# rvp-group/srrg2_slam_interfaces

Measured on AMD Instinct MI355X. Metric: icp_iterations_per_sec, higher is better.
Workload: dtype f32; 1 GPU; C2: SE(3) point-to-plane AlignerSlice, 100000-pt synthetic cloud pair per GPU, 10 ICP iterations per compute(), gated NN 0.25 m + normal gate, Cauchy 0.05; points=100000, alignments_total=1, all_success=True, last_status=0, last_num_inliers=99432, parallelism=single GPU

## Files before the change

### srrg2_slam_interfaces_amd/csrc/aligner_host.hip

```cpp
#include <algorithm>
#include <cmath>
#include <cstdio>
#include <cstdlib>
#include <chrono>
#include <cstring>
#include <string>
#include <vector>

#include "det_math.h"
#include "kernels.h"

#include "host_util.h"

namespace srrg2amd {
thread_local std::string g_err;
int fail(int code, const std::string& msg) {
  g_err = msg;
  return code;
}
}

namespace {

using srrg2amd::DevBuf;
// ... 57 lines not shown
  DevBuf<unsigned long long> zbuf;
  DevBuf<int> queue;
  DevBuf<int> qcount;
  float prior_Z[12]{};
  bool has_prior = false;
  void release() {
    if (qprobe_host) (void) hipHostFree(qprobe_host);
    qprobe_host = nullptr;
    qprobe_cap  = 0;
    if (bbox_host) (void) hipHostFree(bbox_host);
    bbox_host     = nullptr;
    bbox_host_cap = 0;
    if (ms_probs_host) (void) hipHostFree(ms_probs_host);
    ms_probs_host     = nullptr;
    ms_probs_host_cap = 0;
    fixed_raw.release(); fixed_nrm_raw.release(); fixed_sorted.release(); fixed_nrm_sorted.release();
    cell_start.release(); cursor.release(); scan_sums.release(); scalars.release(); pos_of.release();
    list_start.release(); list_sums.release(); list_ent.release(); list_box.release(); list_offs.release(); list_hdr.release();
    moving.release(); moving_nrm.release(); pinf.release();
    moving_raw.release(); moving_nrm_raw.release(); ms_counts.release(); ms_cursor.release(); ms_sums.release();
    ms_bb.release(); ms_probs.release();
    corr_fixed.release(); gcorr.release(); gcorr_off.release(); gcorr_stat.release(); prev_n.release(); prev_pos.release(); prev_f.release(); prev_m.release(); corr_resp.release(); corr_stat.release(); partials.release(); zbuf.release(); queue.release(); qcount.release(); bbox_rows.release();
  }
};

}

struct srrg2_aligner_s {
  int kind = 0, dim = 3, dof = 6, tsize = 12, device = 0;
  hipStream_t stream = nullptr;
  static constexpr int MAX_PARTS = 8;
  hipStream_t pstream[MAX_PARTS]{};
  int cu_count          = 256;
  int fused_grid_max    = 130000;
  hipEvent_t ev_staged  = nullptr;
  hipEvent_t ev_records = nullptr;
  bool records_unsynced = false;
  int parts_dirty       = 0;
  int batch_parts       = 0;
  int part_begin[MAX_PARTS + 1]{};
  srrg2_aligner_params params{10, 10, 0, 0};
  srrg2_reduce_fn reduce_fn = nullptr;
  void* reduce_user         = nullptr;
  long long shard_total     = 0;
  bool has_term = false;
  srrg2_termination_params term{5, 20, 20, 20, 0.2f};
  std::vector<Slice*> slices;
  float X[12]{};
  int status = SRRG2_FAIL;
  int K = 1;
  DevBuf<ProblemDev> probs;
  DevBuf<ProblemState> states;
  DevBuf<ProblemOut> outs;
  DevBuf<srrg2_iteration_stats> stats;
  DevBuf<float> guesses;
  DevBuf<unsigned long long> pub;
  DevBuf<unsigned> pub_epoch;
  DevBuf<CtlParams> ctl_dev;
  DevBuf<char> staging;
  DevBuf<float4> pair_raw, pair_nrm_raw, pair_sorted, pair_nrm_sorted;
  DevBuf<int> pair_cell_start, pair_cursor, pair_scan_sums, pair_pos_of;
  DevBuf<unsigned> pair_rows;
  DevBuf<ProblemDev> pair_fprobs;
  DevBuf<GridDev> pair_grids;
  DevBuf<char> pair_staging;
  unsigned* pair_rows_host = nullptr; size_t pair_rows_host_cap = 0;
// ... 662 lines not shown
  const srrg2_aligner_tuning& tn = a->tuning;
  C.probe_it      = tn.queue_probe_iteration;
  if (a->params.max_iterations <= C.probe_it + 3 || K > 4) C.probe_it = -1;
  bool small = false;
  {
    int ncue = 0, fc = -1;
    for (int si = 0; si < nslices; ++si)
      if (a->slices[si]->cfg.kind != SRRG2_SLICE_PRIOR) {
        if (fc < 0) fc = si;
        ++ncue;
      }
    const int small_max = tn.small_max_points;
    small = ncue == 1 && a->slices[fc]->cfg.finder == SRRG2_FINDER_NN_GATED && max_nm <= small_max &&
            a->timeline_path.empty() && !a->reduce_fn;
    const bool priors_launch = nslices > ncue && (tn.fused_control == 2 || nslices - ncue > 2);
    if (small && !pairs && (priors_launch || tn.fused_control == 0 || a->params.max_iterations < 2)) small = max_nm <= 640;
    if (small && !pairs && !(priors_launch || tn.fused_control == 0 || a->params.max_iterations < 2)) {
      const Slice* sfc = a->slices[fc];
      const int sl     = tn.search_lists;
      const bool lists = sl >= 2 || (sl == 1 && K > 4) || (sl < 0 && (K > 4 || sfc->grid_computes >= 1 || sfc->lists_tried));
      small            = !lists && max_nm <= 384;
    }
  }
  const int fast_from = tn.fast_from_iteration;
  bool fuse = false;
  auto fast_ppt_of = [&](int k_launch) {
    return tn.fast_points_per_thread > 0 ? tn.fast_points_per_thread : (k_launch >= (fuse ? 16 : 64) ? 2 : 1);
  };
  const int fast_min = tn.fast_min_points;
  const bool fast_gather = tn.fast_gather >= 0 ? tn.fast_gather != 0 : K > 4;
  const bool fast_batch_queue = tn.fast_batch_queue != 0;
  const int lds_tile = pairs ? 0 : (tn.lds_tile >= 0 ? tn.lds_tile : (K > 4 ? 1 : 0));
  const int search_lists = tn.search_lists;
  const int search_team_knob = tn.search_team;
  std::vector<char> cnl((size_t) std::max(nslices, 1), 0);
  std::vector<SliceDev> sdev((size_t) nslices);
  int first_cue = -1;
  for (int si = 0; si < nslices; ++si) {
    Slice* s     = a->slices[si];
    SliceCtl& sc = C.slices[si];
    sc.kind                     = s->cfg.kind;
    sc.min_num_correspondences  = s->cfg.min_num_correspondences;
    sc.robust_kind              = s->cfg.robustifier;
    sc.robust_thr               = s->cfg.robustifier_chi_threshold;
    sc.gate                     = s->cfg.finder_max_distance;
    sc.has_prior                = s->has_prior ? 1 : 0;
    sc.prior_sets_initial_guess = s->cfg.prior_sets_initial_guess;
    std::memcpy(sc.prior_Z, s->prior_Z, sizeof(sc.prior_Z));
    std::memcpy(sc.prior_info, s->cfg.prior_information_diag, sizeof(sc.prior_info));
    sc.partials  = nullptr;
    sc.finder    = s->cfg.finder;
    sc.K0        = s->cfg.camera_matrix[0];
    sc.K4        = s->cfg.camera_matrix[4];
    sc.umax      = proj_extent(s->cfg.image_cols, s->cfg.camera_matrix[2]);
    sc.vmax      = proj_extent(s->cfg.image_rows, s->cfg.camera_matrix[5]);
    sc.depth_min = s->cfg.depth_min;
    sc.pinf_bits = nullptr;
    sc.ninf_bits = nullptr;
    if (s->cfg.kind == SRRG2_SLICE_PRIOR) continue;
    if (first_cue < 0) first_cue = si;
    int nm_max_s = 0;
    for (int k = 0; k < K; ++k) nm_max_s = std::max(nm_max_s, all[(size_t) si * K + k].nm);
    const int queue_min = tn.queue_min_points;
    const bool want_lists = search_lists >= 2 || (search_lists == 1 && K > 4) ||
                            (search_lists < 0 && (K > 4 || s->grid_computes >= 1 || s->lists_tried));
    if (!pairs) s->grid_computes++;
    if (s->cfg.finder == SRRG2_FINDER_NN_GATED && !small && want_lists && !pairs) {
// ... 450 lines not shown
                                     a->states.p, K, nm_max, a->stream);
          sdev[si].zbuf_parity ^= 1;
        } else {
          SliceDev sd = sdev[si];
          const bool fast = (slot0 > 0 || (it >= fast_from && it >= 1)) && nm_max >= fast_min;
          if (!queue_on[si] || (s->fast_queue_only && !fast)) {
            sd.queue  = nullptr;
            sd.qcount = nullptr;
          }
          for (int h = 0; h < nhalves; ++h) {
            sd.prob0 = h0[h];
            if (fuse) {
              if (!fused_pass(slot0, it)) sd.fc.pub = nullptr;
              sd.fc.ctl   = a->ctl_dev.p + h;
              sd.fc.epoch = epoch;
              sd.partials = slot_buffer(s, pround);
              sd.fc.prev_partials = slot_buffer(s, pround + 2);
              sd.fc.zero_partials = slot_buffer(s, pround + 1);
              sd.fc.prior         = (slot0 > 0 || it > 0) ? 1 : 0;
              if (it == 0) sd.fc.prior_mask = 0;
            }
            const ProblemDev* pt = a->probs.p + (size_t) si * K;
            hipStream_t hs = hstream[h];
            const int Kh   = hn[h];
            const bool first_pass_init = fold_init && slot0 == 0 && it == 0 && si == first_cue;
            if (pairs && fast)
              srrg2amd::launch_icp_step_fast_pairs(a->dim, plane, sd, pair_grids, pt, a->states.p, Kh, nm_max, fast_ppt_of(Kh),
                                                   fast_gather, hs);
            else if (pairs)
              srrg2amd::launch_icp_step_pairs(a->dim, plane, sd, pair_grids, pt, a->states.p, Kh, nm_max, hs);
            else if (fast)
              srrg2amd::launch_icp_step_fast(a->dim, plane, sd, pt, a->states.p, Kh, nm_max, fast_ppt_of(Kh), fast_gather, hs);
            else if (cnl[(size_t) si] && !sd.queue)
              srrg2amd::launch_icp_step_cnl(a->dim, plane, sd, s->lists_host, pt, a->states.p, Kh, nm_max,
                                            search_team_knob > 0 ? search_team_knob : ((K <= 4 && slot0 == 0 && it == 0) ? 4 : 1), hs,
                                            first_pass_init ? &Ch[h] : nullptr, first_pass_init ? &fold_inl : nullptr,
                                            first_pass_init && !fold_bat.empty() ? &fold_bat[(size_t) h] : nullptr);
            else if (!sd.queue && lds_tile > 0 && !small)
              srrg2amd::launch_icp_step_tile(a->dim, plane, sd, pt, a->states.p, Kh, nm_max, lds_tile == 2 ? 504 : 416, hs);
            else
              srrg2amd::launch_icp_step(a->dim, plane, sd, pt, a->states.p, Kh, nm_max, hs, first_pass_init ? &Ch[h] : nullptr,
                                        first_pass_init ? &fold_inl : nullptr);
            if (split) control(it, last_phase, h);
          }
        }
        if (a->profile) HIP_TRY(hipEventRecord(e1, a->stream));
      }
      if (!split) control(it, last_phase, 0);
      ++epoch;
      ++pround;
    }
    return 0;
  };
  if (small) {
    final_launched = true;
  } else {
    if ((rc = run_phase(0, !a->params.enable_inlier_only_runs))) return rc;
    if (a->params.enable_inlier_only_runs) {
      for (int h = 0; h < nhalves; ++h) {
        Ch[h].epoch = epoch + 1;
        srrg2amd::launch_icp_post(Ch[h], a->states.p, a->stats.p, hstream[h]);
      }
      ++epoch;
      if ((rc = run_phase(a->params.max_iterations, true))) return rc;
    }
  }
  if (!final_launched)
    for (int h = 0; h < nhalves; ++h)
      srrg2amd::launch_icp_finalize(Ch[h], a->states.p, a->stats.p, a->outs_host, a->stats_host,
                                    !a->params.enable_inlier_only_runs , hstream[h]);
// ... 256 lines not shown
  c->finder_normal_cos = -2.f;
  c->finder_cell_size = 0.f;
  identity(variable_kind, c->sensor_in_robot);
  for (int i = 0; i < 6; ++i) c->prior_information_diag[i] = variable_kind == SRRG2_SE2_RIGHT ? 100.f : 1.f;
  c->prior_sets_initial_guess = 1;
}

int srrg2_aligner_create(int variable_kind, int device, srrg2_aligner_h* out) {
  if (!out || variable_kind < 0 || variable_kind > 2) return fail(SRRG2_E_INVALID, "create: bad arguments");
  int n = 0;
  hipError_t e = hipGetDeviceCount(&n);
  if (e != hipSuccess || n <= 0)
    return fail(SRRG2_E_NO_DEVICE, "create: no HIP device visible (this library has no CPU fallback)");
  if (device < 0 || device >= n) return fail(SRRG2_E_INVALID, "create: bad device ordinal");
  srrg2_aligner* a = new srrg2_aligner();
  a->kind   = variable_kind;
  a->dim    = variable_kind == SRRG2_SE2_RIGHT ? 2 : 3;
  a->dof    = variable_kind == SRRG2_SE2_RIGHT ? 3 : 6;
  a->tsize  = variable_kind == SRRG2_SE2_RIGHT ? 9 : 12;
  a->device = device;
  identity(variable_kind, a->X);
  tuning_from_environment(&a->tuning);
  if (const char* tl = std::getenv("SRRG2_AMD_TIMELINE")) a->timeline_path = tl;
  a->hosttime = std::getenv("SRRG2_AMD_HOSTTIME") != nullptr;
  if (const char* fg = std::getenv("SRRG2_AMD_FUSED_GRID_MAX")) a->fused_grid_max = std::atoi(fg);
  bool ok = hipSetDevice(device) == hipSuccess && hipStreamCreateWithFlags(&a->stream, hipStreamNonBlocking) == hipSuccess;
  a->pstream[0] = a->stream;
  ok = ok && hipEventCreateWithFlags(&a->ev_staged, hipEventDisableTiming) == hipSuccess;
  ok = ok && hipEventCreateWithFlags(&a->ev_records, hipEventDisableTiming) == hipSuccess;
  if (ok && (hipDeviceGetAttribute(&a->cu_count, hipDeviceAttributeMultiprocessorCount, device) != hipSuccess || a->cu_count <= 0)) {
    (void) hipGetLastError();
    a->cu_count = 256;
  }
  if (!ok) {
    for (int p = 0; p < srrg2_aligner::MAX_PARTS; ++p)
      if (a->pstream[p]) (void) hipStreamDestroy(a->pstream[p]);
    delete a;
    return fail(SRRG2_E_HIP, "create: cannot create stream");
  }
  *out = a;
  return 0;
}

int srrg2_aligner_destroy(srrg2_aligner_h a) {
  if (!a) return 0;
  (void) hipSetDevice(a->device);
  for (int p = 0; p < srrg2_aligner::MAX_PARTS; ++p)
    if (a->pstream[p]) (void) hipStreamSynchronize(a->pstream[p]);
  for (Slice* s : a->slices) {
    s->release();
    delete s;
  }
  a->probs.release(); a->states.release(); a->outs.release(); a->stats.release(); a->guesses.release();
  a->pub.release(); a->pub_epoch.release(); a->ctl_dev.release();
  a->staging.release();
  a->pair_raw.release(); a->pair_nrm_raw.release(); a->pair_sorted.release(); a->pair_nrm_sorted.release();
  a->pair_cell_start.release(); a->pair_cursor.release(); a->pair_scan_sums.release(); a->pair_pos_of.release();
  a->pair_rows.release(); a->pair_fprobs.release(); a->pair_grids.release(); a->pair_staging.release();
  if (a->pair_rows_host) (void) hipHostFree(a->pair_rows_host);
  if (a->pair_fprobs_host) (void) hipHostFree(a->pair_fprobs_host);
  if (a->pair_grids_host) (void) hipHostFree(a->pair_grids_host);
  if (a->outs_host) (void) hipHostFree(a->outs_host);
  if (a->stats_host) (void) hipHostFree(a->stats_host);
  if (a->guesses_host) (void) hipHostFree(a->guesses_host);
  if (a->probs_host) (void) hipHostFree(a->probs_host);
  for (auto& ev : a->prof_events) {
// ... 818 lines not shown
```

### srrg2_slam_interfaces_amd/csrc/kernels.h

```cpp
#pragma once
#include "device_types.h"

namespace srrg2amd {

void launch_ingest(const float* src, int stride_floats, int n, int dim, float4* dst, unsigned* maxabs_bits,
                   int finite_per_point, hipStream_t s);
void launch_ingest_batch(const float* src, int stride_floats, const ProblemDev* probs, int K, int max_nm, int dim,
                         float4* dst, unsigned* maxabs_bits, int finite_per_point, hipStream_t s);
void launch_bbox(const float4* pts, int n, unsigned* mn, unsigned* mx, int* nvalid, hipStream_t s);
void launch_ingest_bbox(const float* src, int stride_floats, int n, int dim, float4* dst, unsigned* maxabs_bits, unsigned* mn,
                        unsigned* mx, int* nvalid, hipStream_t s, unsigned* ticket, unsigned* host_out, unsigned seq,
                        unsigned* block_out , unsigned* clear_after);
#define INGEST_BBOX_MAX_BLOCKS 512
void launch_grid_count(const GridDev& g, const float4* pts, int n, int* counts, hipStream_t s);
void launch_count_nonzero(const int* counts, int n, int* out, hipStream_t s);
int scan_num_blocks(int n);
void launch_exclusive_scan(int* data, int n, int* block_sums, int* grand_total, hipStream_t s, int* copy = nullptr);
void launch_grid_scatter(const GridDev& g, const float4* pts, const float4* nrm, int n, int* cursor, float4* out_pts,
                         float4* out_nrm, int* pos_of, hipStream_t s);
void launch_cnl_build(const GridDev& g, const GridLists& L, const int4* offs, int noffs, int* list_start, uint2* box_at,
                      uint4* ent, hipStream_t s);
void launch_icp_step_cnl(int dim, bool plane, const SliceDev& S, const GridLists& GL, const ProblemDev* probs,
                         ProblemState* states, int K, int max_nm, int team, hipStream_t s, const CtlParams* init_C = nullptr,
                         const InitInline* init_inl = nullptr, const InitBatch* init_bat = nullptr);
bool launch_msort_local(const float* src, int sf, const float* nsrc, int nsf, const ProblemDev* probs, int K, int dim, int kbits,
                        int aniso, int segments, int max_nm, float4* out_pts, float4* out_nrm, unsigned* maxabs_bits,
                        hipStream_t s);
void launch_msort(const float4* pts, const float4* nrm, const ProblemDev* probs, int K, int max_nm, int kbits, int aniso,
                  unsigned* bb, int* counts, int* cursor, int* scan_sums, int* scan_total, float4* out_pts,
                  float4* out_nrm, hipStream_t s);
void launch_icp_step(int dim, bool plane, const SliceDev& S, const ProblemDev* probs, ProblemState* states, int K,
                     int max_nm, hipStream_t s, const CtlParams* init_C = nullptr, const InitInline* init_inl = nullptr);
void launch_icp_step_tile(int dim, bool plane, const SliceDev& S, const ProblemDev* probs, ProblemState* states, int K,
                          int max_nm, int cap, hipStream_t s);
void launch_icp_step_fast(int dim, bool plane, const SliceDev& S, const ProblemDev* probs, ProblemState* states, int K,
                          int max_nm, int ppt, bool gather, hipStream_t s);
void launch_icp_outputs(int dim, bool plane, const SliceDev& S, const ProblemDev* probs, const ProblemState* states, int K,
                        int max_nm, hipStream_t s);
int icp_step_blocks(int max_nm);
int icp_queue_blocks(int max_nm, int K);
void launch_proj_step_pack(const SliceDev* slices, const ProblemDev* const* probs, int nslices, ProblemState* states, int K,
                           int max_nm, hipStream_t s);
void launch_proj_records(const SliceDev& S0, const SliceDev& S, const ProblemDev* probs0, const ProblemDev* probs,
                         ProblemState* states, int K, int max_nm, bool rebuild, hipStream_t s);
void launch_proj_step_fused(const SliceDev* slices, const ProblemDev* const* probs, int nslices, ProblemState* states, int K,
                            int max_nm, hipStream_t s,
                            const CtlParams* init_C = nullptr, const InitInline* init_inl = nullptr, ProblemDev* probs_base = nullptr);
void launch_corr_step(int dim, bool plane, const SliceDev& S, const ProblemDev* probs, ProblemState* states, int K,
                      int max_ncorr, hipStream_t s);
void launch_proj_step(bool repro, const SliceDev& S, const ProblemDev* probs, ProblemState* states, int K, int max_nm,
                      hipStream_t s);
void launch_icp_init(const CtlParams& C, const ProblemDev* probs_host, ProblemDev* probs, ProblemState* states,
                     const float* guesses_host, int tsize, hipStream_t s, bool pairs = false);
bool make_init_inline(const CtlParams& C, const ProblemDev* probs_host, const float* guesses_host, int tsize, InitInline* inl);
void launch_icp_control(const CtlParams& C, ProblemState* states, srrg2_iteration_stats* stats, hipStream_t s);
void launch_icp_final_wave_pack(const SliceDev* slices, const ProblemDev* const* probs, int nslices, ProblemState* states,
                                srrg2_iteration_stats* stats, ProblemOut* outs_host, srrg2_iteration_stats* stats_host,
// ... 25 lines not shown
```

### srrg2_slam_interfaces_amd/csrc/kernels.hip

```cpp
#include <cstdlib>
#include <algorithm>

#include "kernels.h"

#include <type_traits>

#include "det_math.h"

#include "device_util.h"

namespace {

#define FX_MAGIC 6755399441055744.0
#define FX_MAGIC_BITS 0x4338000000000000ll
__device__ __forceinline__ long long fx_bits(double biased) { return __double_as_longlong(biased) - FX_MAGIC_BITS; }

__device__ __forceinline__ unsigned long long key_min(unsigned long long a, unsigned long long b) {
  double r;
  asm("v_min_f64 %0, %1, %2" : "=v"(r) : "v"(__longlong_as_double((long long) a)), "v"(__longlong_as_double((long long) b)));
  return (unsigned long long) __double_as_longlong(r);
}

template <int DIM>
__device__ __forceinline__ float cand_d2(const float4 f, float qx, float qy, float qz) {
  const float dx = f.x - qx, dy = f.y - qy;
  float d2       = dx * dx + dy * dy;
  if (DIM == 3) {
    const float dz = f.z - qz;
    d2             = d2 + dz * dz;
  }
  return d2;
}

template <int DIM>
__device__ __forceinline__ void test_candidate(const float4 f, float qx, float qy, float qz, bool valid,
                                               unsigned long long& bkey) {
// ... 1705 lines not shown
    }
    const int team = lane >> 4;
    const int mine = team == 0 ? src[0] : (team == 1 ? src[1] : (team == 2 ? src[2] : src[3]));
    const int from = mine >= 0 ? mine : lane;
    float wbest, wexcl2;
    int widx, wpos;
    const int sr_from = __shfl(r2, from);
    coop_scan<DIM, 16>(g, lane, wlds[wid].coop, __shfl(qx, from), __shfl(qy, from), __shfl(qz, from), __shfl(cx, from),
                       __shfl(cy, from), __shfl(cz, from), mine >= 0 ? sr_from : -1, __shfl(ball2, from), wbest, widx, wpos,
                       wexcl2);
#pragma unroll
    for (int t = 0; t < 4; ++t) {
      const float rb = __shfl(wbest, 16 * t), re = __shfl(wexcl2, 16 * t);
      const int ri = __shfl(widx, 16 * t);
      if (lane == src[t]) {
        excl_wide = sqrtf(re) * 0.99999f;
        if (rb < best || (rb == best && ri < bidx)) {
          best = rb;
          bidx = ri;
        }
      }
    }
  }
  if (excl_wide != 0.f || r2 != 0) excl = excl_wide;
  long long acc[ACC_N];
#pragma unroll
  for (int a = 0; a < ACC_N; ++a) acc[a] = 0;
  finish_point<DIM, PLANE>(S, T, rk, thr, kk, scale, inrange, active, gi, oi, p, qx, qy, qz, best, bidx, bpos, excl, skipped,
                           pf, pn, pnm, use_prior && S.use_normal_gate, acc);
  block_reduce_store<NW>(acc, S.partials, prob, tile, nullptr);
}

#ifdef SRRG2_PASS_TIMELINE
__device__ unsigned long long g_pass_ts[16 * 512 * 8];
#define PASS_TS_ANY(epoch, k)                       \
  do {                                                                                                 \
    if ((threadIdx.x & 63) == 0 && (epoch) >= 0 && (epoch) < 16 && blockIdx.y < 512 && blockIdx.x == 0) \
      g_pass_ts[(((epoch) * 512) + blockIdx.y) * 8 + (k)] = wall_clock64();                            \
  } while (0)
#define PASS_TS_W(epoch, k, dep)              \
  do {                                                                                                 \
    if (threadIdx.x == 0 && (epoch) >= 0 && (epoch) < 16 && blockIdx.x == 0) {                         \
      unsigned long long t_ = wall_clock64();                                                          \
      if ((dep) != (dep)) t_ = 0;         \
      g_pass_ts[(((epoch) * 512) + 0) * 8 + (k)] = t_;                                                  \
    }                                                                                                  \
  } while (0)
#define PASS_TS(epoch, k)                                                                              \
  do {                                                                                                 \
    if (threadIdx.x == 0 && (epoch) >= 0 && (epoch) < 16 && blockIdx.y < 512 && blockIdx.x == 0)       \
      g_pass_ts[(((epoch) * 512) + blockIdx.y) * 8 + (k)] = wall_clock64();                            \
  } while (0)
#else
#define PASS_TS(epoch, k) do { } while (0)
#define PASS_TS_ANY(epoch, k) do { } while (0)
#define PASS_TS_W(epoch, k, dep) do { } while (0)
#endif
namespace {

__device__ float robust_weight(int kind, float thr, float chi, bool& kernelized);
template <bool PAIRS = false>
__device__ __forceinline__ int slice_exponent(const CtlParams& C, const SliceCtl& s, int prob, int nm, const float* X);
template <bool ONLY_INLINE, bool PAIRS = false>
__device__ __forceinline__ void init_problem_thread0(const CtlParams& C, int prob, const ProblemDev* probs_host, ProblemDev* probs,
                                                     ProblemState* states, const float* guesses_host, int tsize,
                                                     const InitInline& inl, unsigned (*init_gran)[PUB_SLICE_GRANULES]);

__device__ __forceinline__ double rl_d(double v, int k) {
  const int lo = __builtin_amdgcn_readlane(__double2loint(v), k);
  const int hi = __builtin_amdgcn_readlane(__double2hiint(v), k);
  return __hiloint2double(hi, lo);
}
__device__ __forceinline__ long long rl_ll(long long v, int k) {
  const int lo = __builtin_amdgcn_readlane((int) (unsigned) v, k);
  const int hi = __builtin_amdgcn_readlane((int) (unsigned) ((unsigned long long) v >> 32), k);
  return (long long) (((unsigned long long) (unsigned) hi << 32) | (unsigned) lo);
}
__device__ __forceinline__ float rl_f(float v, int k) { return __int_as_float(__builtin_amdgcn_readlane(__float_as_int(v), k)); }
__device__ __forceinline__ double wave_max_d(double v) {
#pragma unroll
  for (int off = 32; off >= 1; off >>= 1) {
    const double o = __shfl_xor(v, off);
    v              = o > v ? o : v;
  }
// ... 1227 lines not shown
        }
      }
    }
  };
  constexpr bool defer = PPT == 1 && FUSED;
  float d_qx = 0.f, d_qy = 0.f, d_qz = 0.f, d_best = INFINITY;
  bool d_valid = false;
#pragma unroll
  for (int k = 0; k < PPT; ++k) {
    const bool active = inr[k] && finite3(p[k].x, p[k].y, p[k].z);
    float qx, qy, qz, px, py, pz;
    transform_point<DIM>(T, p[k], qx, qy, qz);
    transform_point<DIM>(Tprev, p[k], px, py, pz);
    const float ex = qx - px, ey = qy - py, ez = qz - pz;
    const float dl   = __builtin_amdgcn_sqrtf((ex * ex + ey * ey) + ez * ez);
    const bool hasp  = __float_as_int(pf[k].w) != NO_MATCH;
    unsigned long long k1 = NO_KEY;
    test_candidate<DIM>(pf[k], qx, qy, qz, true, k1);
    const float best = key_best(k1);
    const float d1   = __builtin_amdgcn_sqrtf(best);
    const float rhs  = pm[k] * 0.99999f;
    const bool ca   = hasp && (d1 * 1.00001f + dl * 1.00001f < rhs);
    const bool cc   = !hasp && pm[k] > 0.f && (gate_r * 1.00001f + dl * 1.00001f < rhs);
    const bool have = active && (ca || cc);
    const float excl = pm[k] * 0.9999999f - dl * 1.00001f;
    const float pad  = fminf(2.f * dl, PAD_CAP * g.h) + PAD_MIN * g.h;
    const float rr   = (d1 + pad) * 1.00001f;
    const float r2box = hasp ? fminf(rr * rr, gfar) : gfar;
    open_ball2[k]     = (active && !have) ? r2box : -1.f;
    any_open |= active && !have;
#ifdef SRRG2_PASS_TIMELINE
    if constexpr (FUSED) {
      if (active && !have && S.fc.epoch >= 0 && S.fc.epoch < 16 && blockIdx.x == 0) {
        unsigned long long* c = &g_pass_ts[((size_t) S.fc.epoch * 512 + 500) * 8];
        const float gap = (pm[k] - d1) / g.h;
        atomicAdd(&c[0], 1ull);
        if (!hasp) atomicAdd(&c[1], 1ull);
        else if (gap < 1e-4f) atomicAdd(&c[2], 1ull);
        else if (gap < 0.0202f) atomicAdd(&c[3], 1ull);
        else atomicAdd(&c[4], 1ull);
        if (dl > 1e-3f * g.h) atomicAdd(&c[5], 1ull);
        if (pm[k] <= 0.f) atomicAdd(&c[6], 1ull);
      }
    }
#endif
    if constexpr (defer) {
      d_qx = qx; d_qy = qy; d_qz = qz; d_best = best; d_valid = have && ca;
    } else if (k == 0) {
      linearize(std::true_type{}, acc, have && ca, p[k], pf[k], pn[k], pnm[k], qx, qy, qz, best);
    } else {
      linearize(std::false_type{}, acc, have && ca, p[k], pf[k], pn[k], pnm[k], qx, qy, qz, best);
    }
    if (have) S.prev_m[gi_[k]] = excl;
  }
  if constexpr (defer) {
    {
      if (__any(any_open)) {
        float sbest[PPT], sexcl[PPT];
        int sidx[PPT], spos[PPT];
        search_open(sbest, sidx, sexcl, spos);
        const bool open = open_ball2[0] >= 0.f;
        const bool same = open && sidx[0] != NO_MATCH && sidx[0] == __float_as_int(pf[0].w);
        if (open && !same) {
          pf[0] = make_float4(0.f, 0.f, 0.f, __int_as_float(NO_MATCH));
          pn[0] = make_float4(0.f, 0.f, 0.f, 0.f);
          if (sidx[0] != NO_MATCH) {
            spos[0] = g.pos_of[sidx[0]];
// ... 78 lines not shown
    transform_point<DIM>(T, p[k], qx, qy, qz);
    if (k == 0)
      linearize(std::true_type{}, acc2, open, p[k], fk, nk, pnm[k], qx, qy, qz, sbest[k]);
    else
      linearize(std::false_type{}, acc2, open, p[k], fk, nk, pnm[k], qx, qy, qz, sbest[k]);
    if (open) {
      S.prev_m[gi_[k]] = sexcl[k];
      if (!same) {
        S.prev_pos[gi_[k]] = sidx[k] != NO_MATCH ? spos[k] : -1;
        if (!GATHER) {
          S.prev_f[gi_[k]] = fk;
          if (PLANE || ngate) S.prev_n[gi_[k]] = nk;
        }
      }
    }
  }
  block_reduce_store_biased<1>(acc2, S.partials, prob, tile, PPT);
  if constexpr (FUSED) PASS_TS_ANY(S.fc.epoch, 4);
  block_reduce_store_biased<4, 2>(acc, S.partials, prob, tile, PPT);
  if constexpr (FUSED) PASS_TS(S.fc.epoch, 3);
}

template <int DIM, bool PLANE, int PPT, bool GATHER, int FUSED>
__global__ __launch_bounds__(256) void k_icp_step_fast(SliceDev S, const ProblemDev* __restrict__ probs,
                                                       ProblemState* __restrict__ states) {
  icp_step_fast_body<DIM, PLANE, PPT, GATHER, FUSED>(S, probs, states);
}
template <int DIM, bool PLANE, int PPT, bool GATHER>
__global__ __launch_bounds__(256) void k_icp_step_fast_pairs(SliceDev S, const GridDev* __restrict__ grids,
                                                             const ProblemDev* __restrict__ probs, ProblemState* __restrict__ states) {
  S.grid = grids[blockIdx.y + S.prob0];
  icp_step_fast_body<DIM, PLANE, PPT, GATHER, 0>(S, probs, states);
}
template <int DIM, bool PLANE, int TEAM, int FUSED>
__device__ __forceinline__ void cnl_pass_body(const SliceDev& S, const GridLists& GL, const ProblemDev* __restrict__ probs,
                                              ProblemState* __restrict__ states, const CtlParams* Ci = nullptr,
                                              const InitInline* inl = nullptr, const InitBatch* bat = nullptr) {
  constexpr int NW  = 4;
  constexpr int PPB = NW * 64 / TEAM;
  const int prob    = (FUSED ? blockIdx.x : blockIdx.y) + S.prob0;
  PassView pv;
  if constexpr (!FUSED) {
    pass_view_legacy(S, &states[prob], pv);
    if (pv.stop) return;
  } else if constexpr (FUSED != 3) {
    PASS_TS(S.fc.epoch, 0);
    fused_control_if_due<DIM, FUSED == 2>(S, states, prob);
  }
  ProblemDev pd;
  if constexpr (FUSED == 3) {
    if (bat)
      pd = bat->pd[prob - Ci->prob0];
    else
      pd = inl->pd[S.slice_idx];
  } else {
    pd = probs[prob];
  }
  const int tile      = FUSED ? blockIdx.y : blockIdx.x;
  const bool tail_wg = FUSED == 3 && tile == (int) gridDim.y - 1;
  if (tile * PPB >= pd.nm && (!FUSED || (FUSED == 3 ? !tail_wg : tile != 0))) return;
  float T[12], Tprev[12];
  double scale;
  int rk;
  bool use_prior;
  if constexpr (!FUSED) {
    load_T(pv.T, T);
    load_T(pv.Tprev, Tprev);
    scale     = dm::pow2(pv.kexp);
    rk        = (pv.phase1 && S.robust_kind != SRRG2_ROBUST_NONE) ? (int) SRRG2_ROBUST_CLAMP : S.robust_kind;
    use_prior = pv.prior;
  } else {
    use_prior = S.fc.prior != 0;
  }
  const float thr    = S.robust_thr;
  const float kk     = S.variable_kind == SRRG2_SE3_QUAT_RIGHT ? 2.f : 1.f;
  const GridDev& g   = S.grid;
  const float gfar = use_prior ? g.gate2_ext : g.gate2;

  __shared__ CnlWave wlds[NW];

  const int i        = tile * PPB + (int) threadIdx.x / TEAM;
  const int lane     = threadIdx.x & 63;
  const int wid      = threadIdx.x >> 6;
  const bool leader  = (threadIdx.x & (TEAM - 1)) == 0;
  const bool inrange = i < pd.nm;
  const int gi       = pd.moff + (inrange ? i : 0);
  float4 p           = make_float4(0.f, 0.f, 0.f, 0.f);
  float4 pf          = make_float4(0.f, 0.f, 0.f, __int_as_float(NO_MATCH));
  float4 pn          = make_float4(0.f, 0.f, 0.f, 0.f);
  float4 pnm         = make_float4(0.f, 0.f, 0.f, 0.f);
  float pm           = 0.f;
  if (inrange) {
    p = S.mpts[gi];
    if (use_prior) {
      pm = S.prev_m[gi];
      if (S.use_normal_gate) pnm = S.mnrm[gi];
      if (S.gather_prev) {
        const int ppos = S.prev_pos[gi];
        if (ppos >= 0 && ppos < S.grid.n) {
          pf = S.grid.pts[ppos];
          if (PLANE || S.use_normal_gate) pn = S.grid.nrm[ppos];
        }
      } else {
        pf = S.prev_f[gi];
        if (PLANE || S.use_normal_gate) pn = S.prev_n[gi];
      }
    }
  }
  if constexpr (FUSED) {
    if constexpr (FUSED == 3) {
      pass_view_init<DIM>(S, *Ci, *inl, prob, pd.nm, pv, bat);
      if (tail_wg && threadIdx.x < 64)
        fused_init_tail(*Ci, *inl, prob, const_cast<ProblemDev*>(probs) - (size_t) S.slice_idx * Ci->K, states, bat, pv, S.slice_idx);
    } else {
      pass_view_fused<DIM, FUSED == 2>(S, states, prob, pv);
    }
    if (pv.stop || tile * PPB >= pd.nm) return;
    load_T(pv.T, T);
    load_T(pv.Tprev, Tprev);
    scale = dm::pow2(pv.kexp);
    rk    = (pv.phase1 && S.robust_kind != SRRG2_ROBUST_NONE) ? (int) SRRG2_ROBUST_CLAMP : S.robust_kind;
  }
  const bool has_prev = __float_as_int(pf.w) != NO_MATCH;
  const bool active   = inrange && finite3(p.x, p.y, p.z);
  float qx = 0.f, qy = 0.f, qz = 0.f;
  float best = INFINITY;
  int bidx = NO_MATCH;
  float excl = 0.f, r2box = INFINITY;
  bool skipped = false;
  if (active) {
    transform_point<DIM>(T, p, qx, qy, qz);
    if (use_prior && has_prev) {
      unsigned long long k1 = NO_KEY;
      test_candidate<DIM>(pf, qx, qy, qz, true, k1);
      float px, py, pz;
      transform_point<DIM>(Tprev, p, px, py, pz);
      const float ex = qx - px, ey = qy - py, ez = qz - pz;
      const float dl = sqrtf((ex * ex + ey * ey) + ez * ez);
      const float d1 = sqrtf(key_best(k1));
      if (d1 * 1.00001f + dl * 1.00001f < pm * 0.99999f) {
        skipped = true;
        best    = key_best(k1);
        bidx    = key_idx(k1);
        excl    = pm * 0.9999999f - dl * 1.00001f;
      } else {
        const float pad = fminf(2.f * dl, PAD_CAP * g.h) + PAD_MIN * g.h;
        const float rr  = (d1 + pad) * 1.00001f;
        r2box           = fminf(rr * rr, gfar);
      }
    } else if (use_prior && !has_prev && pm > 0.f) {
// ... 98 lines not shown
    if (!use_prior && found) nmk = S.mnrm[gi];
    float dot;
    if constexpr (DIM == 3) {
      const float rx = (T[0] * nmk.x + T[1] * nmk.y) + T[2] * nmk.z;
      const float ry = (T[4] * nmk.x + T[5] * nmk.y) + T[6] * nmk.z;
      const float rz = (T[8] * nmk.x + T[9] * nmk.y) + T[10] * nmk.z;
      dot            = (nf.x * rx + nf.y * ry) + nf.z * rz;
    } else {
      const float rx = T[0] * nmk.x + T[1] * nmk.y;
      const float ry = T[4] * nmk.x + T[5] * nmk.y;
      dot            = nf.x * rx + nf.y * ry;
    }
    found = found && dot > S.normal_cos;
  }
  long long acc[ACC_N];
  {
    float J[ROWS][D], er[ROWS];
    point_rows<DIM, PLANE>(T, kk, p, qx, qy, qz, fm, nf, J, er);
    (void) factor_accumulate_flat<D, ROWS, true>(J, er, found, rk, thr, scale, acc);
  }
  if (inrange && leader) {
    if (!skipped) {
      S.prev_pos[gi] = has ? bpos : -1;
      if (!S.gather_prev) {
        S.prev_f[gi] = fm;
        if (PLANE || ngate) S.prev_n[gi] = nf;
      }
    }
    S.prev_m[gi] = excl;
  }
  block_reduce_store_biased<NW>(acc, S.partials, prob, tile, 1);
  if constexpr (FUSED) PASS_TS(S.fc.epoch, 3);
}
template <int DIM, bool PLANE, int TEAM, int FUSED>
__global__ __launch_bounds__(256) void k_icp_step_cnl(SliceDev S, GridLists GL, const ProblemDev* __restrict__ probs,
                                                      ProblemState* __restrict__ states) {
  cnl_pass_body<DIM, PLANE, TEAM, FUSED>(S, GL, probs, states);
}
template <int DIM, bool PLANE, int TEAM>
__global__ __launch_bounds__(256) void k_icp_step_cnl_init(SliceDev S, GridLists GL, CtlParams C, InitInline inl,
                                                           ProblemDev* __restrict__ probs, ProblemState* __restrict__ states) {
  cnl_pass_body<DIM, PLANE, TEAM, 3>(S, GL, probs, states, &C, &inl);
}
template <int DIM, bool PLANE, int TEAM>
__global__ __launch_bounds__(256) void k_icp_step_cnl_init_batch(SliceDev S, GridLists GL, CtlParams C, InitBatch B,
                                                                 ProblemDev* __restrict__ probs, ProblemState* __restrict__ states) {
  const InitInline none{};
  cnl_pass_body<DIM, PLANE, TEAM, 3>(S, GL, probs, states, &C, &none, &B);
}

template <int DIM, bool PLANE>
__global__ __launch_bounds__(256) void k_icp_outputs(SliceDev S, const ProblemDev* __restrict__ probs,
                                                     const ProblemState* __restrict__ states) {
  constexpr int D    = DIM == 3 ? 6 : 3;
  constexpr int ROWS = PLANE ? 1 : DIM;
  const int prob     = blockIdx.y + S.prob0;
  const ProblemState* st = &states[prob];
  const ProblemDev pd    = probs[prob];
  const int i            = blockIdx.x * blockDim.x + threadIdx.x;
  if (i >= pd.nm) return;
  const int gi  = pd.moff + i;
  int match     = -1;
  float resp    = 0.f;
  uint8_t fstat = SRRG2_FACTOR_SUPPRESSED;
  const float4 p = S.mpts[gi];
  if (st->npasses > 0 && finite3(p.x, p.y, p.z)) {
    float4 f = make_float4(0.f, 0.f, 0.f, __int_as_float(NO_MATCH));
    int fpos = -1;
    if (S.gather_prev) {
      fpos = S.prev_pos[gi];
      if (fpos >= 0 && fpos < S.grid.n) f = S.grid.pts[fpos];
    } else {
      f = S.prev_f[gi];
    }
    if (__float_as_int(f.w) != NO_MATCH) {
      float T[12];
      load_T(st->Tlast[S.slice_idx], T);
      float qx, qy, qz;
      transform_point<DIM>(T, p, qx, qy, qz);
      unsigned long long k1 = NO_KEY;
      test_candidate<DIM>(f, qx, qy, qz, true, k1);
// ... 1523 lines not shown
    static unsigned long long zero[N];
    if (hipMemcpyToSymbol(HIP_SYMBOL(counters), zero, sizeof(zero)) != hipSuccess) return -1;
  }
  return 0;
}
#endif
#ifdef SRRG2_PASS_TIMELINE
extern "C" int srrg2_amd_debug_pass_timeline(unsigned long long* out, int reset) {
  return debug_counters(g_pass_ts, out, reset);
}
#endif
#ifdef SRRG2_CNL_STATS
extern "C" int srrg2_amd_debug_cnl_stats(unsigned long long* out, int reset) {
  return debug_counters(g_cnl_stats, out, reset);
}
#endif
#ifdef SRRG2_TILE_STATS
extern "C" int srrg2_amd_debug_tile_stats(unsigned long long* out, int reset) {
  return debug_counters(g_tile_stats, out, reset);
}
#endif

void launch_icp_step_tile(int dim, bool plane, const SliceDev& S, const ProblemDev* probs, ProblemState* states, int K,
                          int max_nm, int cap, hipStream_t s) {
  if (K <= 0 || max_nm <= 0) return;
  const dim3 grid(icp_step_blocks(max_nm), K);
  with_dim_plane(dim, plane, [&](auto D, auto P) {
    with_value<504, 416>(cap > 450, [&](auto CAP) {
      hipLaunchKernelGGL((k_icp_step_tile<D(), P(), CAP()>), grid, dim3(256), 0, s, S, probs, states);
    });
  });
}

void launch_icp_step_cnl(int dim, bool plane, const SliceDev& S, const GridLists& GL, const ProblemDev* probs,
                         ProblemState* states, int K, int max_nm, int team, hipStream_t s, const CtlParams* init_C,
                         const InitInline* init_inl, const InitBatch* init_bat) {
  if (K <= 0) return;
  ProblemDev* pw = const_cast<ProblemDev*>(probs);
  auto tiles_of = [&](auto TEAM) { return (max_nm * TEAM() + 255) / 256; };
  if (S.fc.pub && init_C && init_bat) {
    with_value<4, 1>(team >= 4, [&](auto TEAM) {
      const dim3 grid(K, tiles_of(TEAM) + 1);
      with_dim_plane(dim, plane, [&](auto D, auto P) {
        hipLaunchKernelGGL((k_icp_step_cnl_init_batch<D(), P(), TEAM()>), grid, dim3(256), 0, s, S, GL, *init_C, *init_bat, pw,
                           states);
      });
    });
    return;
  }
  if (S.fc.pub && init_C) {
    with_value<4, 1>(team >= 4, [&](auto TEAM) {
      const dim3 grid(K, tiles_of(TEAM) + 1);
      with_dim_plane(dim, plane, [&](auto D, auto P) {
        hipLaunchKernelGGL((k_icp_step_cnl_init<D(), P(), TEAM()>), grid, dim3(256), 0, s, S, GL, *init_C, *init_inl, pw,
                           states);
      });
    });
    return;
  }
  if (max_nm <= 0) return;
  auto pass = [&](auto FUSED) __attribute__((always_inline)) {
    with_value<4, 1>(team >= 4, [&](auto TEAM) {
      const dim3 grid = FUSED() ? dim3(K, tiles_of(TEAM)) : dim3(tiles_of(TEAM), K);
      with_dim_plane(dim, plane, [&](auto D, auto P) {
        hipLaunchKernelGGL((k_icp_step_cnl<D(), P(), TEAM(), FUSED()>), grid, dim3(256), 0, s, S, GL, probs, states);
      });
    });
  };
  if (S.fc.pub && S.fc.prior_mask)
    pass(int_c<2>{});
  else if (S.fc.pub)
    pass(int_c<1>{});
  else
    pass(int_c<0>{});
}

void launch_icp_step_fast(int dim, bool plane, const SliceDev& S, const ProblemDev* probs, ProblemState* states, int K,
                          int max_nm, int ppt, bool gather, hipStream_t s) {
  if (K <= 0 || max_nm <= 0) return;
  auto pass = [&](auto PPT, auto GATHER, auto FUSED) __attribute__((always_inline)) {
    const int tiles = (max_nm + 256 * PPT() - 1) / (256 * PPT());
    const dim3 grid = FUSED() ? dim3(K, tiles) : dim3(tiles, K);
    with_dim_plane(dim, plane, [&](auto D, auto P) {
      hipLaunchKernelGGL((k_icp_step_fast<D(), P(), PPT(), GATHER(), FUSED()>), grid, dim3(256), 0, s, S, probs, states);
    });
  };
  if (S.fc.pub && S.fc.prior_mask) {
    with_value<true, false>(gather, [&](auto G) { pass(int_c<1>{}, G, int_c<2>{}); });
    return;
  }
  if (S.fc.pub) {
    with_value<true, false>(gather, [&](auto G) {
      with_value<2, 1>(ppt >= 2, [&](auto PPT) { pass(PPT, G, int_c<1>{}); });
    });
    return;
  }
  with_value<true, false>(gather, [&](auto G) {
    if (ppt >= 4)
      pass(int_c<4>{}, G, int_c<0>{});
    else
      with_value<2, 1>(ppt >= 2, [&](auto PPT) { pass(PPT, G, int_c<0>{}); });
  });
  if (S.queue) launch_icp_queue(dim, plane, S, probs, states, K, max_nm, s);
}

void launch_icp_outputs(int dim, bool plane, const SliceDev& S, const ProblemDev* probs, const ProblemState* states, int K,
                        int max_nm, hipStream_t s) {
// ... 162 lines not shown
```

Before: 59320 iterations/s.

## Plan mixed-team search tiles to fill resident GPU capacity per ICP iteration

Adds a tile planner that splits the correspondence-search grid into tiles with 4, 2, or 1 lanes per point. It sizes the split against the number of resident workgroups, taken from an occupancy query, so the whole pass fits in one wave of blocks. The automatic lane choice now uses 2-lane teams for early iterations beyond the first, where it previously used 1-lane teams. The aim is better GPU utilisation for single-problem 100k-point searches, at the cost of extra template instantiations, more branching, and an occupancy query at setup.

```diff
diff --git a/srrg2_slam_interfaces_amd/csrc/aligner_host.hip b/srrg2_slam_interfaces_amd/csrc/aligner_host.hip
--- a/srrg2_slam_interfaces_amd/csrc/aligner_host.hip
+++ b/srrg2_slam_interfaces_amd/csrc/aligner_host.hip
@@ -113,6 +113,7 @@
   static constexpr int MAX_PARTS = 8;
   hipStream_t pstream[MAX_PARTS]{};
   int cu_count          = 256;
+  srrg2amd::SearchCapacity search_capacity;
   int fused_grid_max    = 130000;
   hipEvent_t ev_staged  = nullptr;
   hipEvent_t ev_records = nullptr;
@@ -841,7 +842,13 @@
   const bool fast_batch_queue = tn.fast_batch_queue != 0;
   const int lds_tile = pairs ? 0 : (tn.lds_tile >= 0 ? tn.lds_tile : (K > 4 ? 1 : 0));
   const int search_lists = tn.search_lists;
-  const int search_team_knob = tn.search_team;
+  const int search_lanes_knob          = tn.search_team & 0xff;
+  const long long search_capacity_knob = tn.search_team >> 8;
+  int first_pass_lanes = 0;
+  auto search_lanes_auto = [&](int run, int it) {
+    if (K > 4 || run != 0) return 1;
+    return it == 0 ? 4 : (it == 1 || (it == 2 && first_pass_lanes == 2)) ? 2 : 1;
+  };
   std::vector<char> cnl((size_t) std::max(nslices, 1), 0);
   std::vector<SliceDev> sdev((size_t) nslices);
   int first_cue = -1;
@@ -1358,10 +1365,16 @@
             else if (fast)
               srrg2amd::launch_icp_step_fast(a->dim, plane, sd, pt, a->states.p, Kh, nm_max, fast_ppt_of(Kh), fast_gather, hs);
             else if (cnl[(size_t) si] && !sd.queue)
-              srrg2amd::launch_icp_step_cnl(a->dim, plane, sd, s->lists_host, pt, a->states.p, Kh, nm_max,
-                                            search_team_knob > 0 ? search_team_knob : ((K <= 4 && slot0 == 0 && it == 0) ? 4 : 1), hs,
-                                            first_pass_init ? &Ch[h] : nullptr, first_pass_init ? &fold_inl : nullptr,
-                                            first_pass_init && !fold_bat.empty() ? &fold_bat[(size_t) h] : nullptr);
+            {
+              const int lanes = search_lanes_knob > 0 ? search_lanes_knob : search_lanes_auto(slot0, it);
+              const int plan_lanes = (K <= 4 && lanes > 1) ? (lanes >= 4 ? 4 : 2) : 0;
+              const int used = srrg2amd::launch_icp_step_cnl(
+                a->dim, plane, sd, s->lists_host, pt, a->states.p, Kh, nm_max, lanes >= 4 ? 4 : 1, hs,
+                first_pass_init ? &Ch[h] : nullptr, first_pass_init ? &fold_inl : nullptr,
+                first_pass_init && !fold_bat.empty() ? &fold_bat[(size_t) h] : nullptr, plan_lanes, search_lanes_knob == 0,
+                search_capacity_knob, &a->search_capacity);
+              if (slot0 == 0 && it == 0) first_pass_lanes = used;
+            }
             else if (!sd.queue && lds_tile > 0 && !small)
               srrg2amd::launch_icp_step_tile(a->dim, plane, sd, pt, a->states.p, Kh, nm_max, lds_tile == 2 ? 504 : 416, hs);
             else
@@ -1684,6 +1697,7 @@
     (void) hipGetLastError();
     a->cu_count = 256;
   }
+  a->search_capacity.cu_count = a->cu_count;
   if (!ok) {
     for (int p = 0; p < srrg2_aligner::MAX_PARTS; ++p)
       if (a->pstream[p]) (void) hipStreamDestroy(a->pstream[p]);
diff --git a/srrg2_slam_interfaces_amd/csrc/kernels.h b/srrg2_slam_interfaces_amd/csrc/kernels.h
--- a/srrg2_slam_interfaces_amd/csrc/kernels.h
+++ b/srrg2_slam_interfaces_amd/csrc/kernels.h
@@ -20,9 +20,14 @@
                          float4* out_nrm, int* pos_of, hipStream_t s);
 void launch_cnl_build(const GridDev& g, const GridLists& L, const int4* offs, int noffs, int* list_start, uint2* box_at,
                       uint4* ent, hipStream_t s);
-void launch_icp_step_cnl(int dim, bool plane, const SliceDev& S, const GridLists& GL, const ProblemDev* probs,
-                         ProblemState* states, int K, int max_nm, int team, hipStream_t s, const CtlParams* init_C = nullptr,
-                         const InitInline* init_inl = nullptr, const InitBatch* init_bat = nullptr);
+struct SearchCapacity {
+  int cu_count = 256;
+  int blocks_per_cu[2][4] = {{-1, -1, -1, -1}, {-1, -1, -1, -1}};
+};
+int launch_icp_step_cnl(int dim, bool plane, const SliceDev& S, const GridLists& GL, const ProblemDev* probs,
+                        ProblemState* states, int K, int max_nm, int team, hipStream_t s, const CtlParams* init_C = nullptr,
+                        const InitInline* init_inl = nullptr, const InitBatch* init_bat = nullptr, int plan_lanes = 0,
+                        bool plan_whole = false, long long plan_capacity = 0, SearchCapacity* cap = nullptr);
 bool launch_msort_local(const float* src, int sf, const float* nsrc, int nsf, const ProblemDev* probs, int K, int dim, int kbits,
                         int aniso, int segments, int max_nm, float4* out_pts, float4* out_nrm, unsigned* maxabs_bits,
                         hipStream_t s);
diff --git a/srrg2_slam_interfaces_amd/csrc/kernels.hip b/srrg2_slam_interfaces_amd/csrc/kernels.hip
--- a/srrg2_slam_interfaces_amd/csrc/kernels.hip
+++ b/srrg2_slam_interfaces_amd/csrc/kernels.hip
@@ -1,7 +1,9 @@
+#include <climits>
 #include <cstdlib>
 #include <algorithm>
 
 #include "kernels.h"
+#include "search_plan.h"
 
 #include <type_traits>
 
@@ -1773,24 +1775,25 @@
 }
 
 #ifdef SRRG2_PASS_TIMELINE
-__device__ unsigned long long g_pass_ts[16 * 512 * 8];
+#define PASS_TS_WGS 2048
+__device__ unsigned long long g_pass_ts[16 * PASS_TS_WGS * 8];
 #define PASS_TS_ANY(epoch, k)                       \
   do {                                                                                                 \
-    if ((threadIdx.x & 63) == 0 && (epoch) >= 0 && (epoch) < 16 && blockIdx.y < 512 && blockIdx.x == 0) \
-      g_pass_ts[(((epoch) * 512) + blockIdx.y) * 8 + (k)] = wall_clock64();                            \
+    if ((threadIdx.x & 63) == 0 && (epoch) >= 0 && (epoch) < 16 && blockIdx.y < PASS_TS_WGS - 1 && blockIdx.x == 0) \
+      g_pass_ts[(((epoch) * PASS_TS_WGS) + blockIdx.y) * 8 + (k)] = wall_clock64();                            \
   } while (0)
 #define PASS_TS_W(epoch, k, dep)              \
   do {                                                                                                 \
     if (threadIdx.x == 0 && (epoch) >= 0 && (epoch) < 16 && blockIdx.x == 0) {                         \
       unsigned long long t_ = wall_clock64();                                                          \
       if ((dep) != (dep)) t_ = 0;         \
-      g_pass_ts[(((epoch) * 512) + 0) * 8 + (k)] = t_;                                                  \
+      g_pass_ts[(((epoch) * PASS_TS_WGS) + 0) * 8 + (k)] = t_;                                                  \
     }                                                                                                  \
   } while (0)
 #define PASS_TS(epoch, k)                                                                              \
   do {                                                                                                 \
-    if (threadIdx.x == 0 && (epoch) >= 0 && (epoch) < 16 && blockIdx.y < 512 && blockIdx.x == 0)       \
-      g_pass_ts[(((epoch) * 512) + blockIdx.y) * 8 + (k)] = wall_clock64();                            \
+    if (threadIdx.x == 0 && (epoch) >= 0 && (epoch) < 16 && blockIdx.y < PASS_TS_WGS - 1 && blockIdx.x == 0)       \
+      g_pass_ts[(((epoch) * PASS_TS_WGS) + blockIdx.y) * 8 + (k)] = wall_clock64();                            \
   } while (0)
 #else
 #define PASS_TS(epoch, k) do { } while (0)
@@ -3084,7 +3087,7 @@
 #ifdef SRRG2_PASS_TIMELINE
     if constexpr (FUSED) {
       if (active && !have && S.fc.epoch >= 0 && S.fc.epoch < 16 && blockIdx.x == 0) {
-        unsigned long long* c = &g_pass_ts[((size_t) S.fc.epoch * 512 + 500) * 8];
+        unsigned long long* c = &g_pass_ts[((size_t) S.fc.epoch * PASS_TS_WGS + PASS_TS_WGS - 1) * 8];
         const float gap = (pm[k] - d1) / g.h;
         atomicAdd(&c[0], 1ull);
         if (!hasp) atomicAdd(&c[1], 1ull);
@@ -3229,10 +3232,11 @@
   S.grid = grids[blockIdx.y + S.prob0];
   icp_step_fast_body<DIM, PLANE, PPT, GATHER, 0>(S, probs, states);
 }
-template <int DIM, bool PLANE, int TEAM, int FUSED>
+template <int DIM, bool PLANE, int TEAM, int FUSED, bool PLANNED = false>
 __device__ __forceinline__ void cnl_pass_body(const SliceDev& S, const GridLists& GL, const ProblemDev* __restrict__ probs,
                                               ProblemState* __restrict__ states, const CtlParams* Ci = nullptr,
-                                              const InitInline* inl = nullptr, const InitBatch* bat = nullptr) {
+                                              const InitInline* inl = nullptr, const InitBatch* bat = nullptr,
+                                              CnlWave* plan_wlds = nullptr, const int plan_tile = 0, const int plan_first = 0) {
   constexpr int NW  = 4;
   constexpr int PPB = NW * 64 / TEAM;
   const int prob    = (FUSED ? blockIdx.x : blockIdx.y) + S.prob0;
@@ -3243,6 +3247,8 @@
   } else if constexpr (FUSED != 3) {
     PASS_TS(S.fc.epoch, 0);
     fused_control_if_due<DIM, FUSED == 2>(S, states, prob);
+  } else {
+    PASS_TS(S.fc.epoch, 0);
   }
   ProblemDev pd;
   if constexpr (FUSED == 3) {
@@ -3253,9 +3259,10 @@
   } else {
     pd = probs[prob];
   }
-  const int tile      = FUSED ? blockIdx.y : blockIdx.x;
+  const int tile      = PLANNED ? plan_tile : (int) (FUSED ? blockIdx.y : blockIdx.x);
+  const auto first_of = [&]() { return PLANNED ? plan_first : tile * PPB; };
   const bool tail_wg = FUSED == 3 && tile == (int) gridDim.y - 1;
-  if (tile * PPB >= pd.nm && (!FUSED || (FUSED == 3 ? !tail_wg : tile != 0))) return;
+  if (first_of() >= pd.nm &&(!FUSED || (FUSED == 3 ? !tail_wg : tile != 0))) return;
   float T[12], Tprev[12];
   double scale;
   int rk;
@@ -3274,9 +3281,15 @@
   const GridDev& g   = S.grid;
   const float gfar = use_prior ? g.gate2_ext : g.gate2;
 
-  __shared__ CnlWave wlds[NW];
-
-  const int i        = tile * PPB + (int) threadIdx.x / TEAM;
+  CnlWave* wlds;
+  if constexpr (PLANNED) {
+    wlds = plan_wlds;
+  } else {
+    __shared__ CnlWave own_wlds[NW];
+    wlds = own_wlds;
+  }
+
+  const int i        = first_of() + (int) threadIdx.x / TEAM;
   const int lane     = threadIdx.x & 63;
   const int wid      = threadIdx.x >> 6;
   const bool leader  = (threadIdx.x & (TEAM - 1)) == 0;
@@ -3312,7 +3325,7 @@
     } else {
       pass_view_fused<DIM, FUSED == 2>(S, states, prob, pv);
     }
-    if (pv.stop || tile * PPB >= pd.nm) return;
+    if (pv.stop || first_of() >= pd.nm) return;
     load_T(pv.T, T);
     load_T(pv.Tprev, Tprev);
     scale = dm::pow2(pv.kexp);
@@ -3477,6 +3490,23 @@
   block_reduce_store_biased<NW>(acc, S.partials, prob, tile, 1);
   if constexpr (FUSED) PASS_TS(S.fc.epoch, 3);
 }
+struct TilePlan {
+  int t4, t2;
+};
+template <int DIM, bool PLANE, int FUSED>
+__device__ __forceinline__ void cnl_pass_tiles(const SliceDev& S, const GridLists& GL, const ProblemDev* __restrict__ probs,
+                                               ProblemState* __restrict__ states, const TilePlan& plan, const CtlParams* Ci = nullptr,
+                                               const InitInline* inl = nullptr, const InitBatch* bat = nullptr) {
+  __shared__ CnlWave wlds[4];
+  const int tile = FUSED ? blockIdx.y : blockIdx.x;
+  const int t4 = plan.t4, t2 = plan.t2;
+  if (tile < t4)
+    cnl_pass_body<DIM, PLANE, 4, FUSED, true>(S, GL, probs, states, Ci, inl, bat, wlds, tile, tile * 64);
+  else if (tile < t4 + t2)
+    cnl_pass_body<DIM, PLANE, 2, FUSED, true>(S, GL, probs, states, Ci, inl, bat, wlds, tile, t4 * 64 + (tile - t4) * 128);
+  else
+    cnl_pass_body<DIM, PLANE, 1, FUSED, true>(S, GL, probs, states, Ci, inl, bat, wlds, tile, t4 * 64 + t2 * 128 + (tile - t4 - t2) * 256);
+}
 template <int DIM, bool PLANE, int TEAM, int FUSED>
 __global__ __launch_bounds__(256) void k_icp_step_cnl(SliceDev S, GridLists GL, const ProblemDev* __restrict__ probs,
                                                       ProblemState* __restrict__ states) {
@@ -3492,6 +3522,17 @@
                                                                  ProblemDev* __restrict__ probs, ProblemState* __restrict__ states) {
   const InitInline none{};
   cnl_pass_body<DIM, PLANE, TEAM, 3>(S, GL, probs, states, &C, &none, &B);
+}
+template <int DIM, bool PLANE, int FUSED>
+__global__ __launch_bounds__(256) void k_icp_step_cnl_plan(SliceDev S, GridLists GL, const ProblemDev* __restrict__ probs,
+                                                           ProblemState* __restrict__ states, TilePlan plan) {
+  cnl_pass_tiles<DIM, PLANE, FUSED>(S, GL, probs, states, plan);
+}
+template <int DIM, bool PLANE>
+__global__ __launch_bounds__(256) void k_icp_step_cnl_init_plan(SliceDev S, GridLists GL, CtlParams C, InitInline inl,
+                                                                ProblemDev* __restrict__ probs, ProblemState* __restrict__ states,
+                                                                TilePlan plan) {
+  cnl_pass_tiles<DIM, PLANE, 3>(S, GL, probs, states, plan, &C, &inl);
 }
 
 template <int DIM, bool PLANE>
@@ -5081,13 +5122,70 @@
   });
 }
 
-void launch_icp_step_cnl(int dim, bool plane, const SliceDev& S, const GridLists& GL, const ProblemDev* probs,
-                         ProblemState* states, int K, int max_nm, int team, hipStream_t s, const CtlParams* init_C,
-                         const InitInline* init_inl, const InitBatch* init_bat) {
-  if (K <= 0) return;
+static long long cnl_plan_capacity(int dim, bool plane, int kind, SearchCapacity& cap) {
+  int& per_cu = cap.blocks_per_cu[plane ? 1 : 0][kind];
+  if (per_cu < 0) {
+    int n = 0;
+    hipError_t e = hipErrorUnknown;
+    with_dim_plane(dim, plane, [&](auto D, auto P) {
+      if (kind == 3)
+        e = hipOccupancyMaxActiveBlocksPerMultiprocessor(&n, k_icp_step_cnl_init_plan<D(), P()>, 256, 0);
+      else if (kind == 2)
+        e = hipOccupancyMaxActiveBlocksPerMultiprocessor(&n, k_icp_step_cnl_plan<D(), P(), 2>, 256, 0);
+      else if (kind == 1)
+        e = hipOccupancyMaxActiveBlocksPerMultiprocessor(&n, k_icp_step_cnl_plan<D(), P(), 1>, 256, 0);
+      else
+        e = hipOccupancyMaxActiveBlocksPerMultiprocessor(&n, k_icp_step_cnl_plan<D(), P(), 0>, 256, 0);
+    });
+    if (e != hipSuccess) {
+      (void) hipGetLastError();
+      n = 0;
+    }
+    per_cu = n > 6 ? n - 1 : n;
+  }
+  return (long long) per_cu * cap.cu_count;
+}
+
+int launch_icp_step_cnl(int dim, bool plane, const SliceDev& S, const GridLists& GL, const ProblemDev* probs,
+                        ProblemState* states, int K, int max_nm, int team, hipStream_t s, const CtlParams* init_C,
+                        const InitInline* init_inl, const InitBatch* init_bat, int plan_lanes, bool plan_whole,
+                        long long plan_capacity, SearchCapacity* cap) {
+  if (K <= 0) return 0;
   ProblemDev* pw = const_cast<ProblemDev*>(probs);
   auto tiles_of = [&](auto TEAM) { return (max_nm * TEAM() + 255) / 256; };
-  if (S.fc.pub && init_C && init_bat) {
+  const bool init_b = S.fc.pub && init_C && init_bat, init_1 = S.fc.pub && init_C && !init_bat;
+  if (plan_lanes > 1 && cap && !init_b && (init_1 || max_nm > 0)) {
+    const int kind = init_1 ? 3 : (S.fc.pub && S.fc.prior_mask) ? 2 : S.fc.pub ? 1 : 0;
+    const long long resident = plan_capacity > 0 ? plan_capacity : cnl_plan_capacity(dim, plane, kind, *cap);
+    const long long room = std::min(resident - (kind == 3 ? K : 0), 65534ll * K);
+    SearchTiles t{0, 0, 0};
+    bool planned = true;
+    if (plan_whole) {
+      planned = false;
+      for (int l = plan_lanes >= 4 ? 4 : 2; l > 1 && !planned; l >>= 1) {
+        t       = plan_search_tiles(max_nm, K, room, l);
+        planned = (l == 4 ? t.t2 + t.t1 : t.t4 + t.t1) == 0;
+      }
+    } else {
+      t = plan_search_tiles(max_nm, K, room, plan_lanes);
+    }
+    const TilePlan tp{t.t4, t.t2};
+    SliceDev Sp = S;
+    if (resident > 0 && resident < (long long) INT_MAX) Sp.fc.first_round = (int) resident;
+    if (planned) with_dim_plane(dim, plane, [&](auto D, auto P) {
+      if (kind == 3)
+        hipLaunchKernelGGL((k_icp_step_cnl_init_plan<D(), P()>), dim3(K, t.tiles() + 1), dim3(256), 0, s, Sp, GL, *init_C,
+                           *init_inl, pw, states, tp);
+      else if (kind == 2)
+        hipLaunchKernelGGL((k_icp_step_cnl_plan<D(), P(), 2>), dim3(K, t.tiles()), dim3(256), 0, s, Sp, GL, probs, states, tp);
+      else if (kind == 1)
+        hipLaunchKernelGGL((k_icp_step_cnl_plan<D(), P(), 1>), dim3(K, t.tiles()), dim3(256), 0, s, Sp, GL, probs, states, tp);
+      else
+        hipLaunchKernelGGL((k_icp_step_cnl_plan<D(), P(), 0>), dim3(t.tiles(), K), dim3(256), 0, s, Sp, GL, probs, states, tp);
+    });
+    if (planned) return t.t4 ? 4 : t.t2 ? 2 : 1;
+  }
+  if (init_b) {
     with_value<4, 1>(team >= 4, [&](auto TEAM) {
       const dim3 grid(K, tiles_of(TEAM) + 1);
       with_dim_plane(dim, plane, [&](auto D, auto P) {
@@ -5095,9 +5193,9 @@
                            states);
       });
     });
-    return;
-  }
-  if (S.fc.pub && init_C) {
+    return 0;
+  }
+  if (init_1) {
     with_value<4, 1>(team >= 4, [&](auto TEAM) {
       const dim3 grid(K, tiles_of(TEAM) + 1);
       with_dim_plane(dim, plane, [&](auto D, auto P) {
@@ -5105,9 +5203,9 @@
                            states);
       });
     });
-    return;
-  }
-  if (max_nm <= 0) return;
+    return 0;
+  }
+  if (max_nm <= 0) return 0;
   auto pass = [&](auto FUSED) __attribute__((always_inline)) {
     with_value<4, 1>(team >= 4, [&](auto TEAM) {
       const dim3 grid = FUSED() ? dim3(K, tiles_of(TEAM)) : dim3(tiles_of(TEAM), K);
@@ -5122,6 +5220,7 @@
     pass(int_c<1>{});
   else
     pass(int_c<0>{});
+  return 0;
 }
 
 void launch_icp_step_fast(int dim, bool plane, const SliceDev& S, const ProblemDev* probs, ProblemState* states, int K,
diff --git a/srrg2_slam_interfaces_amd/csrc/search_plan.h b/srrg2_slam_interfaces_amd/csrc/search_plan.h
--- /dev/null
+++ b/srrg2_slam_interfaces_amd/csrc/search_plan.h
@@ -0,0 +1,44 @@
+#pragma once
+
+namespace srrg2amd {
+
+struct SearchTiles {
+  int t4, t2, t1;
+  int tiles() const { return t4 + t2 + t1; }
+  long long first_point(int tile) const {
+    if (tile < t4) return 64ll * tile;
+    if (tile < t4 + t2) return 64ll * t4 + 128ll * (tile - t4);
+    return 64ll * t4 + 128ll * t2 + 256ll * (tile - t4 - t2);
+  }
+};
+
+inline SearchTiles plan_search_tiles(int max_nm, int K, long long capacity_wgs, int lanes_cap) {
+  const long long n  = max_nm > 0 ? max_nm : 0;
+  const long long T1 = (n + 255) / 256;
+  SearchTiles one{0, 0, (int) T1};
+  if (n == 0 || K <= 0 || lanes_cap < 2) return one;
+  const long long T = capacity_wgs / K;
+  if (T1 > T) return one;
+  SearchTiles p{0, 0, 0};
+  long long left = n, tiles = T;
+  if (lanes_cap >= 4) {
+    if ((n + 63) / 64 <= T) return SearchTiles{(int) ((n + 63) / 64), 0, 0};
+    long long t = (256 * tiles - left) / 192;
+    if (t > left / 64) t = left / 64;
+    p.t4 = (int) t;
+    left -= 64 * t;
+    tiles -= t;
+  }
+  if ((left + 127) / 128 <= tiles) {
+    p.t2 = (int) ((left + 127) / 128);
+    return p;
+  }
+  long long t = (256 * tiles - left) / 128;
+  if (t > left / 128) t = left / 128;
+  p.t2 = (int) t;
+  left -= 128 * t;
+  p.t1 = (int) ((left + 255) / 256);
+  return p;
+}
+
+}
```

Result: faster. 60750 iterations/s (median of 6 runs) (+2.4%).
